# encryptorion-lab/phantom-fhe

Measured on AMD Instinct MI355X. Metric: forward NTT limb-transforms/s at N=2^16, 45 RNS moduli, higher is better.
Workload: dtype u64; 1 GPU; CKKS N=2^16, 45 data limbs (+15 special), forward NTT of a batch of 16 ciphertext polynomials per step (720 limb-transforms, 360 MiB, HBM-resident; configs[2] parameter set); N=65536, limbs=45, special_limbs=15, parallelism=ciphertext-batch x1, launch=K steps enqueued by one library call (2 K eager kernel launches)

## Files before the change

### phantom-fhe_amd/csrc/pha_ntt.hip

```cpp
#include "../../include/phantom_amd.h"
#include "pha_internal.h"
#include "pha_experiments.h"
#include "pha_ntt_core.h"

#include <atomic>
#include <type_traits>
#include <cstdlib>

namespace pha {

#ifndef PHA_X_HOIST_C
#define PHA_X_HOIST_C 0
#endif
#ifndef PHA_X_HOIST_S
#define PHA_X_HOIST_S 0
#endif
#ifndef PHA_X_VARIANT
#define PHA_X_VARIANT (1 | 32 | 64 | 2048 | 4096)
#endif
constexpr int kDefaultVariant = PHA_X_VARIANT;
#if defined(PHA_EXPERIMENTS)
std::atomic<int> g_ntt_variant{kDefaultVariant};
static inline int ntt_variant() { return g_ntt_variant.load(std::memory_order_relaxed); }
std::atomic<int> g_whole14_min{1 << 30};
std::atomic<int> g_fused_split{0};
std::atomic<int> g_fused_lag{2};
std::atomic<int> g_fused_min_tiles{1 << 30};
extern std::atomic<int> g_bconv_split;
#else
static constexpr int ntt_variant() { return kDefaultVariant; }
#endif
#if defined(PHA_EXP_STAMPS)
__device__ unsigned long long g_stamps[8];
__device__ unsigned long long g_wg_times[2048];
#endif

struct NttKArgs {
    const u64 *in;
    u64 *out;
    u64 *mid;
    const u64x2 *tw;
    const DModulus *mod;
    const u64x2 *ninv;
    const u64x2 *w1ninv;
    const u64 *twf;
    const u64x2 *ninvf, *w1ninvf;
    const FpInfo *fpinfo;
    const u64 *scale;
    const u64 *scale_shoup;
    const u64 *aux;
    const u64 *aux2;
    const u64 *scale2, *scale2_shoup;
    size_t aux2_stride;
    LimbSel sel;
    uint32_t log_n;
    uint32_t t1, t2;
    uint32_t active;
    uint32_t batch;
    size_t poly_stride, out_stride, aux_stride;
    size_t in_stride;
    bool first_pass_only;
    bool second_pass_only;
    bool first_pass_done;
    uint32_t excl_step, excl_limit, excl_mod;
    const u64 *pro_src;
    size_t pro_stride;
    uint32_t zfast_tiles;
    uint32_t zfast_run;
    u64 pro_t;
    size_t aux_pair_stride;
    const u64 *h_primes;
};

template <bool FWD, int EPI, bool FOLD>
__device__ __forceinline__ void tile_args(const NttKArgs &k, uint32_t twr, uint32_t tile, PassArgs &a) {
    const uint32_t prime = twr >= k.sel.remap_from ? twr + k.sel.remap_add : twr;
    const size_t n = (size_t)1 << k.log_n;
    a.in = k.in + (size_t)twr * n;
    a.out = k.out + (size_t)twr * n;
    a.tw = k.tw + (size_t)prime * n;
    a.twd = nullptr;
    a.q = k.mod[prime].value;
    a.tile = tile;
    a.rho0 = k.t1;
    a.stride = k.t2;
    if (!FWD && FOLD) {
        a.ninv = k.ninv[prime];
        a.w1ninv = k.w1ninv[prime];
    }
    a.pro_reduce = false;
    a.pro_ratio1 = 0;
    a.fp = false;
    if (k.fpinfo) {
        const FpInfo fi = k.fpinfo[prime];
        if (fi.ok) {
            a.fp = true;
            a.fpm = FpMod{fi.q, fi.qinv, (fi.ok & 2) != 0, (fi.ok & 4) != 0};
            a.twd = k.twf + (size_t)prime * n;
            if (!FWD && FOLD) {
                a.ninv = k.ninvf[prime];
                a.w1ninv = k.w1ninvf[prime];
// ... 6 lines not shown
    }
    a.aux = (EPI == EPI_FWD_MODDOWN || EPI == EPI_FWD_MODDOWN_ADD || EPI == EPI_FWD_KSRESCALE || EPI == EPI_INV_CANON_ADD) ? k.aux + (size_t)twr * n : nullptr;
    if (EPI == EPI_FWD_KSRESCALE) {
        a.scale2.x = k.scale2[twr];
        a.scale2.y = k.scale2_shoup[twr];
        a.aux2 = k.aux2 + (size_t)twr * n;
    }
}

#if defined(PHA_PASS_OCC)
#define PHA_PASS_ATTR __attribute__((amdgpu_waves_per_eu(PHA_PASS_OCC, PHA_PASS_OCC)))
#else
#define PHA_PASS_ATTR
#endif
#if defined(PHA_EXP_STAMPS)
#define PHA_STAMP(i) do { if (blockIdx.x == 0 && blockIdx.y == 0 && threadIdx.x == 0) g_stamps[i] = __builtin_readcyclecounter(); } while (0)
#else
#define PHA_STAMP(i) do { } while (0)
#endif

__device__ __forceinline__ bool limb_excluded(const NttKArgs &k, uint32_t twr, uint32_t z) {
    const uint32_t zd = k.excl_mod ? z % k.excl_mod : z;
    const uint32_t es = k.sel.excl_start + zd * k.excl_step;
    uint32_t ee = es + (k.sel.excl_end - k.sel.excl_start);
    ee = ee < k.excl_limit ? ee : k.excl_limit;
    return twr >= es && twr < ee;
}

template <class C, bool FWD, int EPI, bool FOLD>
__device__ __forceinline__ void full_tile_args(const NttKArgs &k, uint32_t twr, uint32_t z, uint32_t tile, PassArgs &a) {
    tile_args<FWD, EPI, FOLD>(k, twr, tile, a);
    if (k.batch > 1) {
        a.in += (size_t)z * k.in_stride;
        a.out += (size_t)z * k.out_stride;
        if (EPI == EPI_FWD_MODDOWN || EPI == EPI_FWD_MODDOWN_ADD || EPI == EPI_FWD_KSRESCALE) a.aux += (size_t)z * k.aux_stride;
        if (EPI == EPI_FWD_KSRESCALE) a.aux2 += (size_t)z * k.aux2_stride;
    }
    if (EPI == EPI_INV_CANON_ADD) a.aux += (size_t)(z >> 1) * k.aux_pair_stride + (size_t)(z & 1) * k.aux_stride;
    if (FWD && (C::STRIDED || C::WHOLE) && k.pro_src) {
        const uint32_t prime = twr >= k.sel.remap_from ? twr + k.sel.remap_add : twr;
        a.in = k.pro_src + (size_t)z * k.pro_stride;
        a.pro_reduce = true;
        a.pro_ratio1 = k.mod[prime].ratio1;
        a.pro_half = bfv_lift_threshold(k.pro_t);
        a.pro_inc = bfv_lift_increment(a.q, k.pro_t);
    }
}

template <class C, bool FWD, int EPI, bool FOLD, int HOIST, bool COH, int ONLY = 0, int PRO = PRO_NONE>
__device__ __forceinline__ void exec_pass(const PassArgs &a, u64 *lds, int tid) {
    u64 reg[C::EPT];
    u64x2 twreg[C::TW_TOTAL];
    using Prog = PassProgram<C, FWD, EPI, FOLD, HOIST, COH, PRO>;
    auto pass = [&](const PassArgs &pa) __attribute__((always_inline)) {
        Prog::load_twiddles(pa, tid, twreg);
        Prog::template run<0>(pa, lds, tid, reg, twreg);
        PHA_STAMP(1);
        tile_sync<C>();
        PHA_STAMP(2);
        Prog::template run<1>(pa, lds, tid, reg, twreg);
        PHA_STAMP(3);
        if constexpr (Prog::NSEG >= 3) {
            tile_sync<C>();
            PHA_STAMP(4);
            Prog::template run<2>(pa, lds, tid, reg, twreg);
            PHA_STAMP(5);
        }
        if constexpr (Prog::NSEG == 4) {
            tile_sync<C>();
            Prog::template run<3>(pa, lds, tid, reg, twreg);
        }
    };
    if (ONLY != 2 && a.fp) {
        PassArgs b = a;
        b.fp = true;
        pass(b);
    } else {
        PassArgs b = a;
        b.fp = false;
        pass(b);
    }
}

struct ZloopMap {
    uint32_t n_int, n_fp;
    uint32_t zper;
    uint32_t tiles;
    uint32_t int_blocks;
    uint8_t limb[128];
};
template <class C, bool FWD, int EPI, bool FOLD>
__global__ __launch_bounds__(C::THREADS) void ntt_zloop_kernel(const NttKArgs k, const ZloopMap m) {
    static_assert(!C::WHOLE, "the batched form exists for the passes of the two-pass plans");
    extern __shared__ __attribute__((aligned(16))) unsigned char smem[];
    u64 *lds = reinterpret_cast<u64 *>(smem);
    __builtin_amdgcn_s_setprio(3);
    const int tid = threadIdx.x;
    uint32_t b = blockIdx.x;
    PassArgs a;
    if (b < m.int_blocks) {
        const uint32_t tile = b % m.tiles, rest = b / m.tiles, z = rest % k.batch, twr = k.sel.start + m.limb[rest / k.batch];
        if (limb_excluded(k, twr, z)) return;
        full_tile_args<C, FWD, EPI, FOLD>(k, twr, z, tile, a);
        exec_pass<C, FWD, EPI, FOLD, 0, false, 2>(a, lds, tid);
        return;
    }
    b -= m.int_blocks;
    const uint32_t tile = b % m.tiles, rest = b / m.tiles, zgroups = (k.batch + m.zper - 1) / m.zper;
    const uint32_t twr = k.sel.start + m.limb[m.n_int + rest / zgroups];
    const uint32_t z0 = (rest % zgroups) * m.zper, z1 = (z0 + m.zper < k.batch) ? z0 + m.zper : k.batch;
    full_tile_args<C, FWD, EPI, FOLD>(k, twr, z0, tile, a);
    using Prog = PassProgram<C, FWD, EPI, FOLD, 1, false>;
    a.fp = true;
    u64x2 twreg[C::TW_TOTAL];
    Prog::load_twiddles(a, tid, twreg);
    u64 regA[C::EPT], regB[C::EPT];
    auto args_of = [&](uint32_t z) __attribute__((always_inline)) {
        PassArgs b = a;
        const size_t dz = (size_t)(z - z0);
        b.in += dz * k.in_stride;
        b.out += dz * k.out_stride;
        if (EPI == EPI_FWD_MODDOWN || EPI == EPI_FWD_MODDOWN_ADD || EPI == EPI_FWD_KSRESCALE) b.aux += dz * k.aux_stride;
        if (EPI == EPI_FWD_KSRESCALE) b.aux2 += dz * k.aux2_stride;
        return b;
    };
    auto transform = [&](const PassArgs &b, u64 *reg) __attribute__((always_inline)) {
        Prog::template run_prefetched<0>(b, lds, tid, reg, twreg);
        tile_sync<C>();
        Prog::template run_prefetched<1>(b, lds, tid, reg, twreg);
        if constexpr (Prog::NSEG >= 3) {
            tile_sync<C>();
            Prog::template run_prefetched<2>(b, lds, tid, reg, twreg);
        }
        if constexpr (Prog::NSEG == 4) {
            tile_sync<C>();
            Prog::template run_prefetched<3>(b, lds, tid, reg, twreg);
        }
        tile_sync<C>();
    };
    auto next = [&](uint32_t z) __attribute__((always_inline)) {
        while (z < z1 && limb_excluded(k, twr, z)) z++;
        return z;
    };
    uint32_t z = next(z0);
    if (z >= z1) return;
    Prog::prefetch(args_of(z), tid, regA);
    __builtin_amdgcn_s_setprio(0);
    for (;;) {
        uint32_t zn = next(z + 1);
        if (zn < z1) Prog::prefetch(args_of(zn), tid, regB);
        transform(args_of(z), regA);
        if (zn >= z1) break;
        z = zn;
        zn = next(z + 1);
        if (zn < z1) Prog::prefetch(args_of(zn), tid, regA);
        transform(args_of(z), regB);
        if (zn >= z1) break;
        z = zn;
    }
}

#if defined(PHA_X_OCC_S) || defined(PHA_X_OCC_C)
#ifndef PHA_X_OCC_S
#define PHA_X_OCC_S 2
#endif
#ifndef PHA_X_OCC_C
#define PHA_X_OCC_C 1
#endif
template <class C> constexpr int x_occ() { return C::WHOLE ? 1 : C::STRIDED ? (C::THREADS >= 512 ? PHA_X_OCC_S : 1) : (C::THREADS == 64 ? PHA_X_OCC_C : 1); }
#define PHA_PASS_BOUNDS __launch_bounds__(C::THREADS, x_occ<C>())
#else
#define PHA_PASS_BOUNDS __launch_bounds__(C::THREADS)
#endif
template <class C, bool FWD, int EPI, bool FOLD, int HOIST, int PRO = PRO_NONE>
__global__ PHA_PASS_BOUNDS PHA_PASS_ATTR void ntt_pass_kernel(const NttKArgs k) {
    extern __shared__ __attribute__((aligned(16))) unsigned char smem[];
    u64 *lds = reinterpret_cast<u64 *>(smem);

    __builtin_amdgcn_s_setprio(3);
    uint32_t tile = blockIdx.x, y = blockIdx.y, z = blockIdx.z;
    if (k.zfast_tiles) {
        const uint32_t b = blockIdx.x, per_chunk = k.zfast_run * k.batch, chunk = b / per_chunk, rem = b - chunk * per_chunk;
        z = rem / k.zfast_run;
        const uint32_t group = chunk * k.zfast_run + (rem - z * k.zfast_run);
        if (group >= k.zfast_tiles * k.sel.count) return;
        tile = group % k.zfast_tiles;
        y = group / k.zfast_tiles;
    }
    const uint32_t twr = k.sel.start + y;
    if (limb_excluded(k, twr, z)) return;
    PassArgs a;
    full_tile_args<C, FWD, EPI, FOLD>(k, twr, z, tile, a);
#if defined(PHA_EXP_STAMPS)
    const unsigned long long wg_t0 = wall_clock64();
#endif
    PHA_STAMP(0);
    exec_pass<C, FWD, EPI, FOLD, HOIST, false, 0, PRO>(a, lds, threadIdx.x);
#if defined(PHA_EXP_STAMPS)
    __builtin_amdgcn_s_waitcnt(0);
    PHA_STAMP(6);
    if (threadIdx.x == 0) {
        const unsigned id = blockIdx.y * gridDim.x + blockIdx.x;
        if (id < 1024) { g_wg_times[2 * id] = wg_t0; g_wg_times[2 * id + 1] = wall_clock64(); }
    }
#endif
}

#if defined(PHA_EXPERIMENTS)
#ifndef PHA_FUSED_MIN_WAVES
#define PHA_FUSED_MIN_WAVES 6
#endif
#if defined(PHA_FUSED_DEBUG)
__device__ uint32_t g_fused_dbg[8];
#endif
struct FusedArgs {
    uint32_t *cls;
    uint32_t *flags;
    uint32_t units, slots, tpl, lag, count;
    uint32_t active_units;
    uint32_t split;
};
__device__ __forceinline__ void l2_arrive(uint32_t *p) {
    asm volatile("global_atomic_add %0, %1, off" ::"v"(p), "v"(1u) : "memory");
}
__device__ __forceinline__ uint32_t l2_fetch_or(uint32_t *p, uint32_t v) {
    uint32_t r;
    asm volatile("global_atomic_or %0, %1, %2, off sc0\n\ts_waitcnt vmcnt(0)" : "=&v"(r) : "v"(p), "v"(v) : "memory");
    return r;
}
__device__ __forceinline__ uint32_t l2_fetch_add(uint32_t *p, uint32_t v) {
    uint32_t r;
    asm volatile("global_atomic_add %0, %1, %2, off sc0\n\ts_waitcnt vmcnt(0)" : "=&v"(r) : "v"(p), "v"(v) : "memory");
    return r;
}
__device__ __forceinline__ void l2_store(uint32_t *p, uint32_t v) {
    asm volatile("global_atomic_swap %0, %1, off" ::"v"(p), "v"(v) : "memory");
}

template <class C, bool FWD, int EPI, bool FOLD, bool COH>
__device__ __forceinline__ void fused_run_tile(const NttKArgs &k, uint32_t twr, uint32_t z, uint32_t tile, u64 *lds) {
    static_assert(C::THREADS == 512 || C::THREADS == 64, "the one-launch transform runs 512-thread workgroups");
    PassArgs a;
    if constexpr (C::THREADS == 512) {
        full_tile_args<C, FWD, EPI, FOLD>(k, twr, z, tile, a);
        exec_pass<C, FWD, EPI, FOLD, 0, COH>(a, lds, threadIdx.x);
    } else {
        const uint32_t wave = threadIdx.x >> 6;
        full_tile_args<C, FWD, EPI, FOLD>(k, twr, z, tile * 8 + wave, a);
        exec_pass<C, FWD, EPI, FOLD, 0, COH>(a, lds + (size_t)wave * C::LDS_WORDS, threadIdx.x & 63);
    }
}

template <class PS, class PC, bool FWD, int EPI, bool FOLD>
__global__ __launch_bounds__(512, PHA_FUSED_MIN_WAVES) void ntt_fused_kernel(const NttKArgs kA, const NttKArgs kB, const FusedArgs f) {
    extern __shared__ __attribute__((aligned(16))) unsigned char smem[];
    u64 *lds = reinterpret_cast<u64 *>(smem);
    const uint32_t b = blockIdx.x, xcd = b & 7u, within = b >> 3;
    const uint32_t role = f.split ? (within & 1u) : 2u, idx = f.split ? (within >> 1) : within;
    const uint32_t tile = idx % f.tpl, slot = idx / f.tpl;
    const uint32_t uA = slot * 8 + xcd;
    const bool has_a = role != 1u && slot < f.slots && uA < f.units && !limb_excluded(kA, kA.sel.start + uA % f.count, uA / f.count);
    const uint32_t uB = (slot - f.lag) * 8 + xcd;
    const bool has_b = role != 0u && slot >= f.lag && uB < f.units && !limb_excluded(kB, kB.sel.start + uB % f.count, uB / f.count);
    if (!has_a && !has_b) return;
    uint32_t cls_seen = 0, cls_mine = 0;
    if (threadIdx.x == 0) {
        uint32_t id;
        asm volatile("s_getreg_b32 %0, hwreg(HW_REG_XCC_ID)" : "=s"(id));
        cls_mine = (id & 7u) + 1;
        uint32_t expected = 0;
        __hip_atomic_compare_exchange_strong(f.cls + xcd, &expected, cls_mine, __ATOMIC_RELAXED, __ATOMIC_RELAXED, __HIP_MEMORY_SCOPE_AGENT);
        cls_seen = expected;
    }
    if (has_a) {
        const uint32_t z = uA / f.count, twr = kA.sel.start + uA % f.count;
        if (FWD) fused_run_tile<PS, true, EPI_NONE, false, false>(kA, twr, z, tile, lds);
        else fused_run_tile<PC, false, EPI_NONE, false, false>(kA, twr, z, tile, lds);
        asm volatile("s_waitcnt vmcnt(0)" ::: "memory");
        __syncthreads();
        if (threadIdx.x == 0) l2_arrive(f.flags + 2 * (size_t)uA);
    }
    if (threadIdx.x == 0 && cls_seen != 0 && cls_seen != cls_mine) {
#if defined(PHA_FUSED_DEBUG)
        if (atomicAdd(&g_fused_dbg[0], 1u) == 0) { g_fused_dbg[1] = b; g_fused_dbg[2] = cls_mine; g_fused_dbg[3] = cls_seen; }
#else
        __builtin_trap();
#endif
    }
    if (!has_b) return;
    const uint32_t z = uB / f.count, twr = kB.sel.start + uB % f.count;
    uint32_t *flag = f.flags + 2 * (size_t)uB;
    constexpr bool kWaveConsumer = FWD && PC::THREADS == 64;
    const bool poller = kWaveConsumer && f.split ? (threadIdx.x & 63) == 0 : threadIdx.x == 0;
    if (poller) {
        uint32_t spins = 0;
        while (l2_fetch_or(flag, 0u) < f.tpl) {
            __builtin_amdgcn_s_sleep(8);
#if defined(PHA_FUSED_DEBUG)
            if (++spins > (1u << 16)) { atomicAdd(&g_fused_dbg[4], 1u); break; }
#else
            if (++spins > (1u << 24)) __builtin_trap();
#endif
        }
    }
    if (!(kWaveConsumer && f.split)) __syncthreads();
    if (FWD) fused_run_tile<PC, true, EPI, false, true>(kB, twr, z, tile, lds);
    else fused_run_tile<PS, false, EPI, FOLD, true>(kB, twr, z, tile, lds);
    __syncthreads();
    if (threadIdx.x == 0 && __hip_atomic_fetch_add(flag + 1, 1u, __ATOMIC_RELAXED, __HIP_MEMORY_SCOPE_WORKGROUP) == f.tpl - 1) {
        l2_store(flag, 0u);
        l2_store(flag + 1, 0u);
        if (__hip_atomic_fetch_add(f.cls + 8, 1u, __ATOMIC_RELAXED, __HIP_MEMORY_SCOPE_AGENT) == f.active_units - 1) {
            for (int i = 0; i < 9; i++) __hip_atomic_store(f.cls + i, 0u, __ATOMIC_RELAXED, __HIP_MEMORY_SCOPE_AGENT);
        }
    }
}

#endif

template <class C, bool FWD, int EPI, bool FOLD, int PRO = PRO_NONE>
static void launch_pass(const NttKArgs &k, hipStream_t s) {
    const size_t n = (size_t)1 << k.log_n;
    const size_t lds_bytes = (size_t)C::LDS_WORDS * sizeof(u64);
    const unsigned tiles_per_limb = (unsigned)(n >> C::LOGTILE);
    dim3 grid(tiles_per_limb, k.sel.count, k.batch);
    NttKArgs kk = k;
    kk.zfast_tiles = 0;
    if (!C::STRIDED && !C::WHOLE && k.zfast_tiles) {
        kk.zfast_tiles = tiles_per_limb;
        kk.zfast_run = 8;
#if defined(PHA_X_KNOBS)
        static const unsigned run_x = std::getenv("PHA_X_ZRUN") ? (unsigned)std::atol(std::getenv("PHA_X_ZRUN")) : 8u;
        kk.zfast_run = run_x;
#endif
        const unsigned groups = tiles_per_limb * k.sel.count;
        grid = dim3(((groups + kk.zfast_run - 1) / kk.zfast_run) * kk.zfast_run * k.batch, 1, 1);
    }
    if (lds_bytes > 64 * 1024) {
        static std::atomic<uint64_t> raised{0};
        int dev = 0;
        PHA_HIP(hipGetDevice(&dev));
        const uint64_t bit = 1ull << (dev & 63);
        if (!(raised.load(std::memory_order_acquire) & bit)) {
            PHA_HIP(hipFuncSetAttribute(reinterpret_cast<const void *>(&ntt_pass_kernel<C, FWD, EPI, FOLD, (C::WHOLE ? 0 : C::STRIDED ? PHA_X_HOIST_S : PHA_X_HOIST_C), PRO>),
                                        hipFuncAttributeMaxDynamicSharedMemorySize, (int)lds_bytes));
            raised.fetch_or(bit, std::memory_order_release);
        }
    }
    constexpr int HX = C::WHOLE ? 0 : C::STRIDED ? PHA_X_HOIST_S : PHA_X_HOIST_C;
#if defined(PHA_X_KNOBS)
    static const size_t pad_s = std::getenv("PHA_X_LDS_S") ? (size_t)std::atol(std::getenv("PHA_X_LDS_S")) : 0;
    static const size_t pad_c = std::getenv("PHA_X_LDS_C") ? (size_t)std::atol(std::getenv("PHA_X_LDS_C")) : 0;
    const size_t lds_x = lds_bytes + (C::STRIDED ? pad_s : pad_c);
    hipLaunchKernelGGL((ntt_pass_kernel<C, FWD, EPI, FOLD, HX, PRO>), grid, dim3(C::THREADS), lds_x, s, kk);
#else
    hipLaunchKernelGGL((ntt_pass_kernel<C, FWD, EPI, FOLD, HX, PRO>), grid, dim3(C::THREADS), lds_bytes, s, kk);
#endif
    check_launch();
}

#if defined(PHA_EXPERIMENTS)
template <class PS, class PC, bool FWD, int EPI, bool FOLD>
static bool launch_fused(Context &c, const NttKArgs &kA_in, const NttKArgs &kB_in, hipStream_t s) {
    static_assert(PS::THREADS == 512 && PS::LOGTILE == 12, "strided pass: one 4096-coefficient tile per 512-thread workgroup");
    NttKArgs kA = kA_in, kB = kB_in;
    const size_t n = (size_t)1 << kA.log_n;
    kA.zfast_tiles = kB.zfast_tiles = 0;
    FusedArgs f{};
    f.count = kA.sel.count;
    f.units = kA.sel.count * kA.batch;
    f.slots = (f.units + 7) / 8;
    f.tpl = (uint32_t)(n >> 12);
    f.lag = (uint32_t)g_fused_lag.load(std::memory_order_relaxed);
    f.cls = c.ntt_flags(s, f.units);
    if (!f.cls) return false;
    f.flags = f.cls + 16;
    f.active_units = 0;
    for (uint32_t z = 0; z < kA.batch; z++) {
        const uint32_t zd = kA.excl_mod ? z % kA.excl_mod : z;
        const uint32_t es = kA.sel.excl_start + zd * kA.excl_step;
        uint32_t ee = es + (kA.sel.excl_end - kA.sel.excl_start);
        ee = ee < kA.excl_limit ? ee : kA.excl_limit;
        const uint32_t lo = es > kA.sel.start ? es : kA.sel.start;
        const uint32_t hi = ee < kA.sel.start + kA.sel.count ? ee : kA.sel.start + kA.sel.count;
        f.active_units += kA.sel.count - (hi > lo ? hi - lo : 0);
    }
    if (f.active_units == 0) return true;
    const size_t lds_a = (size_t)PS::LDS_WORDS * sizeof(u64);
    const size_t lds_b = (size_t)PC::LDS_WORDS * sizeof(u64) * (PC::THREADS == 64 ? 8 : 1);
    const size_t lds_bytes = lds_a > lds_b ? lds_a : lds_b;
    f.split = g_fused_split.load(std::memory_order_relaxed) ? 1u : 0u;
    const unsigned blocks = (f.slots + f.lag) * f.tpl * 8 * (f.split ? 2u : 1u);
    hipLaunchKernelGGL((ntt_fused_kernel<PS, PC, FWD, EPI, FOLD>), dim3(blocks), dim3(512), lds_bytes, s, kA, kB, f);
    check_launch();
    return true;
}

#endif

template <class P>
static void launch_inverse_last(const NttKArgs &k, int epi, hipStream_t s) {
    if (epi == EPI_INV_SCALE) launch_pass<P, false, EPI_INV_SCALE, true>(k, s);
    else if (epi == EPI_INV_CANON_ADD) launch_pass<P, false, EPI_INV_CANON_ADD, true>(k, s);
    else launch_pass<P, false, EPI_INV_CANON, true>(k, s);
}

template <class W>
static void forward_whole(NttKArgs k, int epi, hipStream_t s) {
    k.t1 = 1;
    k.t2 = W::T;
    k.mid = k.out;
    if (epi == EPI_FWD_MODDOWN) launch_pass<W, true, EPI_FWD_MODDOWN, false>(k, s);
    else if (epi == EPI_FWD_MODDOWN_ADD) launch_pass<W, true, EPI_FWD_MODDOWN_ADD, false>(k, s);
    else if (epi == EPI_FWD_KSRESCALE) launch_pass<W, true, EPI_FWD_KSRESCALE, false>(k, s);
    else if (k.pro_t) launch_pass<W, true, EPI_FWD_CANON, false, PRO_LIFT>(k, s);
    else launch_pass<W, true, EPI_FWD_CANON, false>(k, s);
}
template <class W>
static void inverse_whole(NttKArgs k, int epi, hipStream_t s) {
    k.t1 = 1;
    k.t2 = W::T;
    k.mid = k.out;
    launch_inverse_last<W>(k, epi, s);
}

#ifndef PHA_ZLOOP_MIN_BATCH
#define PHA_ZLOOP_MIN_BATCH 8
#endif
template <class C, bool FWD, int EPI, bool FOLD>
static bool launch_zloop(const NttKArgs &k, hipStream_t s) {
    if (k.batch < (uint32_t)PHA_ZLOOP_MIN_BATCH || k.pro_src) return false;
    const size_t n = (size_t)1 << k.log_n;
    const unsigned tiles_per_limb = (unsigned)(n >> C::LOGTILE);
    const size_t waves_per_poly = (size_t)tiles_per_limb * k.sel.count * (C::THREADS / 64);
    const size_t want = (size_t)256 * 4 * 4 * 3;
    uint32_t zper = (k.batch + ((k.batch + 7) / 8) - 1) / ((k.batch + 7) / 8);
    while (zper > 4 && waves_per_poly * ((k.batch + zper - 1) / zper) < want) zper = (zper + 1) / 2;
    if (waves_per_poly * ((k.batch + zper - 1) / zper) < want / 3) return false;
#if defined(PHA_X_KNOBS)
    static const unsigned zper_x = std::getenv("PHA_X_ZPER") ? (unsigned)std::atol(std::getenv("PHA_X_ZPER")) : 0u;
    if (zper_x) zper = zper_x;
#endif
    auto is_fp = [&](uint32_t y) {
        const uint32_t twr = k.sel.start + y, prime = twr >= k.sel.remap_from ? twr + k.sel.remap_add : twr;
        return k.fpinfo != nullptr && (k.h_primes[prime] >> 50) == 0;
    };
    if (k.sel.count > 128) return false;
    ZloopMap m{};
    m.zper = zper;
    m.tiles = tiles_per_limb;
    for (uint32_t y = 0; y < k.sel.count; y++)
        if (!is_fp(y)) m.limb[m.n_int++] = (uint8_t)y;
    for (uint32_t y = 0; y < k.sel.count; y++)
        if (is_fp(y)) m.limb[m.n_int + m.n_fp++] = (uint8_t)y;
    if (m.n_fp * 2 < k.sel.count) return false;
    m.int_blocks = m.n_int * tiles_per_limb * k.batch;
    NttKArgs kk = k;
    kk.zfast_tiles = 0;
    const unsigned blocks = m.int_blocks + m.n_fp * tiles_per_limb * ((k.batch + zper - 1) / zper);
    const size_t lds_bytes = (size_t)C::LDS_WORDS * sizeof(u64);
    hipLaunchKernelGGL((ntt_zloop_kernel<C, FWD, EPI, FOLD>), dim3(blocks), dim3(C::THREADS), lds_bytes, s, kk, m);
    check_launch();
    return true;
}

#ifndef PHA_IP_PLAN
#define PHA_IP_PLAN 3
#endif
template <int LOGN, int VARIANT>
static void forward_impl(NttKArgs k, int epi, hipStream_t s, Context *fused = nullptr) {
    using P1 = typename NttPlan<LOGN, VARIANT>::P1;
    using P2 = typename NttPlan<LOGN, VARIANT>::P2;
    k.t1 = P1::T;
    k.t2 = P2::T;
    if (k.first_pass_done && !(LOGN == 16 && VARIANT == 10 && P1::LOGT == 6))
        throw std::logic_error("ntt_forward: first_pass_done needs the 64 x 1024 plan the fused conversion wrote");
    u64 *const final_out = k.out;
    const size_t final_stride = k.out_stride;
    k.out = k.mid;
    k.out_stride = k.poly_stride;
    const NttKArgs k1 = k;
    k.in = k.mid;
    k.in_stride = k.poly_stride;
    k.out = final_out;
    k.out_stride = final_stride;
    k.pro_src = nullptr;
#if defined(PHA_EXPERIMENTS)
    if constexpr (P1::THREADS == 512 && P1::LOGTILE == 12 && P2::THREADS == 64) {
        if (fused && epi != EPI_FWD_KSRESCALE && !k.first_pass_done && !k.pro_t) {
            const bool done = epi == EPI_FWD_MODDOWN ? launch_fused<P1, P2, true, EPI_FWD_MODDOWN, false>(*fused, k1, k, s)
                              : epi == EPI_FWD_MODDOWN_ADD ? launch_fused<P1, P2, true, EPI_FWD_MODDOWN_ADD, false>(*fused, k1, k, s)
                                                           : launch_fused<P1, P2, true, EPI_FWD_CANON, false>(*fused, k1, k, s);
            if (done) return;
        }
    }
#else
    (void)fused;
#endif
    if (k.first_pass_done) {
    } else if (k1.pro_t) launch_pass<P1, true, EPI_NONE, false, PRO_LIFT>(k1, s);
    else launch_pass<P1, true, EPI_NONE, false>(k1, s);
    if (k.first_pass_only) return;
#if !defined(PHA_NO_ZLOOP)
    if constexpr (VARIANT == 10 || VARIANT == 3 || VARIANT == 4) {
        using Z2 = typename NttPlan<LOGN, VARIANT == 4 ? 3 : VARIANT>::P2;
        const bool done = epi == EPI_FWD_MODDOWN ? launch_zloop<Z2, true, EPI_FWD_MODDOWN, false>(k, s)
                          : epi == EPI_FWD_MODDOWN_ADD ? launch_zloop<Z2, true, EPI_FWD_MODDOWN_ADD, false>(k, s)
                          : epi == EPI_FWD_KSRESCALE ? launch_zloop<Z2, true, EPI_FWD_KSRESCALE, false>(k, s)
                                                     : launch_zloop<Z2, true, EPI_FWD_CANON, false>(k, s);
        if (done) return;
    }
#endif
    if (epi == EPI_FWD_MODDOWN) launch_pass<P2, true, EPI_FWD_MODDOWN, false>(k, s);
    else if (epi == EPI_FWD_MODDOWN_ADD) launch_pass<P2, true, EPI_FWD_MODDOWN_ADD, false>(k, s);
    else if (epi == EPI_FWD_KSRESCALE) launch_pass<P2, true, EPI_FWD_KSRESCALE, false>(k, s);
    else launch_pass<P2, true, EPI_FWD_CANON, false>(k, s);
}

template <int LOGN, int VARIANT>
static void inverse_impl(NttKArgs k, int epi, hipStream_t s, Context *fused = nullptr) {
    using P1 = typename NttPlan<LOGN, VARIANT>::P1;
    using P2 = typename NttPlan<LOGN, VARIANT>::P2;
    k.t1 = P1::T;
    k.t2 = P2::T;
    u64 *const final_out = k.out;
    const size_t final_stride = k.out_stride;
    k.out = k.mid;
    k.out_stride = k.poly_stride;
    const NttKArgs k1 = k;
    k.in = k.mid;
    k.in_stride = k.poly_stride;
    k.out = final_out;
    k.out_stride = final_stride;
#if defined(PHA_EXPERIMENTS)
    if constexpr (P1::THREADS == 512 && P1::LOGTILE == 12 && P2::THREADS == 64) {
        if (fused && epi != EPI_INV_CANON_ADD) {
            const bool done = epi == EPI_INV_SCALE ? launch_fused<P1, P2, false, EPI_INV_SCALE, true>(*fused, k1, k, s)
                                                   : launch_fused<P1, P2, false, EPI_INV_CANON, true>(*fused, k1, k, s);
            if (done) return;
        }
    }
#else
    (void)fused;
#endif
    if (k.second_pass_only) {
        using IpPlan = NttPlan<LOGN, (LOGN >= 14 && LOGN <= 16) ? PHA_IP_PLAN : 3>;
        if (P1::LOGT + IpPlan::P2::LOGT != LOGN)
            throw std::logic_error("second_pass_only: the chosen plan's strided pass does not complete the fused mod-up's contiguous pass");
        launch_inverse_last<P1>(k, epi, s);
        return;
    }
#if !defined(PHA_NO_ZLOOP)
    if constexpr (VARIANT == 10 || VARIANT == 3 || VARIANT == 4) {
        using Z2 = typename NttPlan<LOGN, VARIANT == 4 ? 3 : VARIANT>::P2;
        if (!launch_zloop<Z2, false, EPI_NONE, false>(k1, s)) launch_pass<P2, false, EPI_NONE, false>(k1, s);
        launch_inverse_last<P1>(k, epi, s);
        return;
    }
#endif
    launch_pass<P2, false, EPI_NONE, false>(k1, s);
    launch_inverse_last<P1>(k, epi, s);
}

static NttKArgs make_args(Context &c, const u64 *in, u64 *mid, u64 *out, const LimbSel &sel, const NttExtra &x,
                          bool fwd) {
    NttKArgs k{};
    k.in = in;
    k.mid = mid;
    k.out = out;
    k.tw = fwd ? c.d_tw.p : c.d_itw.p;
    k.mod = c.d_mod.p;
    k.ninv = c.d_ninv.p;
    k.w1ninv = c.d_w1ninv.p;
    const bool use_fp = !(ntt_variant() & 8);
    k.twf = fwd ? c.d_twf.p : c.d_itwf.p;
    k.ninvf = c.d_ninvf.p;
    k.w1ninvf = c.d_w1ninvf.p;
    k.fpinfo = use_fp ? c.d_fpinfo.p : nullptr;
    k.scale = x.scale;
    k.scale_shoup = x.scale_shoup;
    k.aux = x.aux;
    k.aux2 = x.aux2;
    k.scale2 = x.scale2;
    k.scale2_shoup = x.scale2_shoup;
    k.aux2_stride = x.aux2_stride ? x.aux2_stride : x.poly_stride;
    k.sel = sel;
    k.log_n = c.log_n;
    k.h_primes = c.primes.data();
    k.batch = x.batch ? x.batch : 1;
    k.poly_stride = x.poly_stride;
    k.in_stride = x.in_stride ? x.in_stride : x.poly_stride;
    k.first_pass_only = fwd && x.first_pass_only;
    k.second_pass_only = !fwd && x.second_pass_only;
    k.first_pass_done = fwd && x.first_pass_done;
    k.out_stride = x.out_stride ? x.out_stride : x.poly_stride;
    k.aux_stride = x.aux_stride ? x.aux_stride : x.poly_stride;
    k.excl_step = x.excl_step;
    k.excl_limit = x.excl_limit;
    k.excl_mod = x.excl_mod;
    k.pro_src = fwd ? x.pro_src : nullptr;
    k.pro_stride = x.pro_stride;
    k.pro_t = fwd && x.pro_src ? x.pro_lift_t : 0;
    k.aux_pair_stride = x.aux_pair_stride;
    uint32_t excl = 0;
    if (sel.excl_end > sel.excl_start) {
        const uint32_t lo = sel.excl_start > sel.start ? sel.excl_start : sel.start;
        const uint32_t hi = sel.excl_end < sel.start + sel.count ? sel.excl_end : sel.start + sel.count;
        excl = hi > lo ? hi - lo : 0;
        if (excl && (lo != sel.excl_start || hi != sel.excl_end)) excl = 0xffffffffu;
    }
    k.active = excl == 0xffffffffu ? 0 : sel.count - excl;
    return k;
}

static void check_sel(Context &c, const LimbSel &sel) {
    if (sel.count == 0) return;
    const uint32_t last = sel.start + sel.count - 1;
    const uint32_t prime_last = last >= sel.remap_from ? last + sel.remap_add : last;
    if (prime_last >= c.rows) throw std::invalid_argument("modulus index out of range of the NTT tables");
}


template <class C, int BETA, bool FP>
__device__ __forceinline__ void modup_ip_body(const NttKArgs &k, const ModupIpArgs &ip, uint32_t twr, uint32_t prime, uint32_t tile,
                                              u64 *lds, int tid) {
    constexpr int RL = C::NR - 1, r = C::r(RL), K = 1 << r, G = C::EPT >> r;
    static_assert(C::LOGT - C::s0(RL) - r == 0, "the last round holds runs of K consecutive coefficients");
    using Prog = PassProgram<C, true, EPI_NONE, false, 0, false>;
    const size_t n = (size_t)1 << k.log_n;
    const DModulus m = k.mod[prime];
    const u64 q = m.value;
    FpMod fm{};
    u64 accb[C::EPT], acca[C::EPT];
#pragma unroll
    for (int i = 0; i < C::EPT; i++) accb[i] = acca[i] = FP ? as_u64(0.0) : 0;
    size_t g0[G];
#pragma unroll
    for (int gi = 0; gi < G; gi++) {
        int v, hi, lo;
// ... 815 lines not shown
```

### phantom-fhe_amd/csrc/pha_ntt_core.h

```cpp
#pragma once
#include "pha_arith.h"
#include "pha_bfv_lift.h"

namespace pha {

constexpr int kTileElems = 4096;

enum Epilogue {
    EPI_NONE = 0,
    EPI_FWD_CANON = 1,
    EPI_FWD_MODDOWN = 2,
    EPI_INV_CANON = 3,
    EPI_INV_SCALE = 4,
    EPI_FWD_MODDOWN_ADD = 5,
    EPI_FWD_KSRESCALE = 6,
    EPI_INV_CANON_ADD = 7,
};

enum Prologue {
    PRO_NONE = 0,
    PRO_LIFT = 1,
};

template <int LOGT_, bool STRIDED_, int R0_, int R1_, int R2_ = 0, int EPT_ = 16, bool OT_ = false, int LOGTILE_ = 12,
// ... 658 lines not shown
        }
#if !defined(PHA_X_NOCOMPUTE)
        round_compute<C, RI, FWD, FOLD && RI == 0, fp_sched().recentre[SEG], fp_sched().full[SEG]>(a, tid, reg, twreg);
#endif
        if (last) fp_before_global_store(a, reg);
        round_out<C, RI, last, last ? EPI : (int)EPI_NONE>(a, lds, tid, reg);
    }

    template <int SEG>
    PHA_HD static void run_keep(const PassArgs &a, u64 *lds, int tid, u64 *reg, u64x2 *twreg) {
        constexpr int RI = FWD ? SEG : C::NR - 1 - SEG;
        static_assert(SEG == C::NR - 1 && SEG > 0, "run_keep is the last segment of a multi-round pass");
        segment_twiddles<SEG>(a, tid, twreg);
        round_load<C, RI, false, COH>(a, lds, tid, reg);
        round_compute<C, RI, FWD, FOLD && RI == 0>(a, tid, reg, twreg);
    }

    static constexpr int RI_FIRST = FWD ? 0 : C::NR - 1;
    PHA_HD static void prefetch(const PassArgs &a, int tid, u64 *reg) {
        round_load<C, RI_FIRST, true>(a, nullptr, tid, reg);
    }
    template <int SEG>
    PHA_HD static void run_prefetched(const PassArgs &a, u64 *lds, int tid, u64 *reg, u64x2 *twreg) {
        constexpr int RI = FWD ? SEG : C::NR - 1 - SEG;
        constexpr bool first = SEG == 0, last = SEG == C::NR - 1;
        segment_twiddles<SEG>(a, tid, twreg);
        if (!first) round_load<C, RI, false>(a, lds, tid, reg);
        if (first) fp_after_global_load(a, reg);
        round_compute<C, RI, FWD, FOLD && RI == 0, fp_sched().recentre[SEG], fp_sched().full[SEG]>(a, tid, reg, twreg);
        if (last) fp_before_global_store(a, reg);
        round_out<C, RI, last, last ? EPI : (int)EPI_NONE>(a, lds, tid, reg);
    }
};

template <int LOGN, int VARIANT> struct NttPlan;
template <> struct NttPlan<12, 0> { using P1 = PassCfg<6, true, 3, 3>;  using P2 = PassCfg<6, false, 3, 3>; };
template <> struct NttPlan<13, 0> { using P1 = PassCfg<6, true, 3, 3>;  using P2 = PassCfg<7, false, 4, 3>; };
template <> struct NttPlan<14, 0> { using P1 = PassCfg<7, true, 4, 3>;  using P2 = PassCfg<7, false, 4, 3>; };
template <> struct NttPlan<15, 0> { using P1 = PassCfg<7, true, 4, 3>;  using P2 = PassCfg<8, false, 4, 4>; };
template <> struct NttPlan<16, 0> { using P1 = PassCfg<8, true, 4, 4>;  using P2 = PassCfg<8, false, 4, 4>; };
template <> struct NttPlan<17, 0> { using P1 = PassCfg<8, true, 4, 4>;  using P2 = PassCfg<9, false, 3, 3, 3>; };
template <> struct NttPlan<12, 1> { using P1 = PassCfg<6, true, 3, 3, 0, 8>;  using P2 = PassCfg<6, false, 3, 3, 0, 8>; };
template <> struct NttPlan<13, 1> { using P1 = PassCfg<6, true, 3, 3, 0, 8>;  using P2 = PassCfg<7, false, 3, 2, 2, 8>; };
template <> struct NttPlan<14, 1> { using P1 = PassCfg<7, true, 3, 2, 2, 8>;  using P2 = PassCfg<7, false, 3, 2, 2, 8>; };
template <> struct NttPlan<15, 1> { using P1 = PassCfg<7, true, 3, 2, 2, 8>;  using P2 = PassCfg<8, false, 3, 3, 2, 8>; };
template <> struct NttPlan<16, 1> { using P1 = PassCfg<8, true, 3, 3, 2, 8>;  using P2 = PassCfg<8, false, 3, 3, 2, 8>; };
template <> struct NttPlan<17, 1> { using P1 = PassCfg<8, true, 3, 3, 2, 8>;  using P2 = PassCfg<9, false, 3, 3, 3, 8>; };
template <> struct NttPlan<12, 2> { using P1 = PassCfg<6, true, 3, 3, 0, 8>;  using P2 = PassCfg<6, false, 3, 3, 0, 8, true>; };
template <> struct NttPlan<13, 2> { using P1 = PassCfg<6, true, 3, 3, 0, 8>;  using P2 = PassCfg<7, false, 3, 2, 2, 8, true>; };
template <> struct NttPlan<14, 2> { using P1 = PassCfg<7, true, 3, 2, 2, 8>;  using P2 = PassCfg<7, false, 3, 2, 2, 8, true>; };
template <> struct NttPlan<15, 2> { using P1 = PassCfg<7, true, 3, 2, 2, 8>;  using P2 = PassCfg<8, false, 3, 3, 2, 8, true>; };
template <> struct NttPlan<16, 2> { using P1 = PassCfg<8, true, 3, 3, 2, 8>;  using P2 = PassCfg<8, false, 3, 3, 2, 8, true>; };
template <> struct NttPlan<17, 2> { using P1 = PassCfg<8, true, 3, 3, 2, 8>;  using P2 = PassCfg<9, false, 3, 3, 3, 8, true>; };
template <> struct NttPlan<12, 3> { using P1 = PassCfg<6, true, 3, 3, 0, 8>;  using P2 = PassCfg<6, false, 3, 3, 0, 8, false, 9>; };
template <> struct NttPlan<13, 3> { using P1 = PassCfg<6, true, 3, 3, 0, 8>;  using P2 = PassCfg<7, false, 3, 2, 2, 8, false, 9>; };
template <> struct NttPlan<14, 3> { using P1 = PassCfg<7, true, 3, 2, 2, 8>;  using P2 = PassCfg<7, false, 3, 2, 2, 8, false, 9>; };
template <> struct NttPlan<15, 3> { using P1 = PassCfg<7, true, 3, 2, 2, 8>;  using P2 = PassCfg<8, false, 3, 3, 2, 8, false, 9>; };
template <> struct NttPlan<16, 3> { using P1 = PassCfg<8, true, 3, 3, 2, 8>;  using P2 = PassCfg<8, false, 3, 3, 2, 8, false, 9>; };
template <> struct NttPlan<17, 3> { using P1 = PassCfg<8, true, 3, 3, 2, 8>;  using P2 = PassCfg<9, false, 3, 3, 3, 8, false, 9>; };
template <> struct NttPlan<12, 4> { using P1 = PassCfg<6, true, 3, 3, 0, 8>;  using P2 = PassCfg<6, false, 3, 3, 0, 8, true, 9>; };
template <> struct NttPlan<13, 4> { using P1 = PassCfg<6, true, 3, 3, 0, 8>;  using P2 = PassCfg<7, false, 3, 2, 2, 8, true, 9>; };
template <> struct NttPlan<14, 4> { using P1 = PassCfg<7, true, 3, 2, 2, 8>;  using P2 = PassCfg<7, false, 3, 2, 2, 8, true, 9>; };
template <> struct NttPlan<15, 4> { using P1 = PassCfg<7, true, 3, 2, 2, 8>;  using P2 = PassCfg<8, false, 3, 3, 2, 8, true, 9>; };
template <> struct NttPlan<16, 4> { using P1 = PassCfg<8, true, 3, 3, 2, 8>;  using P2 = PassCfg<8, false, 3, 3, 2, 8, true, 9>; };
template <> struct NttPlan<17, 4> { using P1 = PassCfg<8, true, 3, 3, 2, 8>;  using P2 = PassCfg<9, false, 3, 3, 3, 8, true, 9>; };
template <> struct NttPlan<14, 5> { using P1 = PassCfg<7, true, 3, 2, 2, 8>;  using P2 = PassCfg<7, false, 2, 2, 2, 4, false, 8, false, 1>; };
template <> struct NttPlan<15, 5> { using P1 = PassCfg<7, true, 3, 2, 2, 8>;  using P2 = PassCfg<8, false, 2, 2, 2, 4, false, 8, false, 2>; };
template <> struct NttPlan<16, 5> { using P1 = PassCfg<8, true, 3, 3, 2, 8>;  using P2 = PassCfg<8, false, 2, 2, 2, 4, false, 8, false, 2>; };
template <> struct NttPlan<14, 6> { using P1 = PassCfg<7, true, 2, 2, 2, 4, false, 11, false, 1>;  using P2 = NttPlan<14, 5>::P2; };
template <> struct NttPlan<15, 6> { using P1 = PassCfg<7, true, 2, 2, 2, 4, false, 11, false, 1>;  using P2 = NttPlan<15, 5>::P2; };
template <> struct NttPlan<16, 6> { using P1 = PassCfg<8, true, 2, 2, 2, 4, false, 11, false, 2>;  using P2 = NttPlan<16, 5>::P2; };
template <> struct NttPlan<14, 7> { using P1 = PassCfg<7, true, 2, 2, 2, 4, false, 12, false, 1>;  using P2 = NttPlan<14, 5>::P2; };
template <> struct NttPlan<15, 7> { using P1 = PassCfg<7, true, 2, 2, 2, 4, false, 12, false, 1>;  using P2 = NttPlan<15, 5>::P2; };
template <> struct NttPlan<16, 7> { using P1 = PassCfg<8, true, 2, 2, 2, 4, false, 12, false, 2>;  using P2 = NttPlan<16, 5>::P2; };
template <> struct NttPlan<16, 8> { using P1 = PassCfg<7, true, 3, 2, 2, 8>;  using P2 = PassCfg<9, false, 3, 3, 3, 8, false, 9>; };
template <> struct NttPlan<16, 9> { using P1 = PassCfg<7, true, 3, 2, 2, 8>;  using P2 = PassCfg<9, false, 3, 3, 3, 8, true, 9>; };
template <> struct NttPlan<16, 10> { using P1 = PassCfg<6, true, 3, 3, 0, 8, false, 11>;  using P2 = PassCfg<10, false, 3, 3, 2, 8, false, 10, false, 2>; };
template <> struct NttPlan<16, 12> { using P1 = PassCfg<6, true, 3, 3, 0, 8>;  using P2 = PassCfg<10, false, 4, 3, 3, 16, false, 10>; };
template <> struct NttPlan<16, 13> { using P1 = PassCfg<6, true, 2, 2, 2, 4, false, 10>;  using P2 = NttPlan<16, 10>::P2; };
using WholePlan12 = PassCfg<12, false, 4, 4, 4, 16, false, 12, true>;
using WholePlan13 = PassCfg<13, false, 4, 4, 4, 16, false, 13, true, 1>;
using WholePlan14 = PassCfg<14, false, 4, 4, 4, 16, false, 14, true, 2>;

}
```

Before: 2.589 million NTT/s.

## Reverse strided-pass block order so the zloop pass reuses cache-resident limbs

Adds a PassOrder descriptor that remaps the first (strided) pass grid so blocks run limbs and batch entries in the reverse of the order the following zloop pass consumes them. The most recently written data is then still in the last-level cache when the second pass starts reading it. An optional mode splits the limbs into two halves when the working set exceeds the cache size, though it is off by default. The cost is an extra kernel argument plus decode work in the pass kernel, and block scheduling may become less balanced.

```diff
diff --git a/phantom-fhe_amd/csrc/pha_ntt.hip b/phantom-fhe_amd/csrc/pha_ntt.hip
--- a/phantom-fhe_amd/csrc/pha_ntt.hip
+++ b/phantom-fhe_amd/csrc/pha_ntt.hip
@@ -17,6 +17,12 @@
 #endif
 #ifndef PHA_X_VARIANT
 #define PHA_X_VARIANT (1 | 32 | 64 | 2048 | 4096)
+#endif
+#ifndef PHA_NTT_PASS_ORDER
+#define PHA_NTT_PASS_ORDER 1
+#endif
+#ifndef PHA_NTT_ORDER_INT_HEAD
+#define PHA_NTT_ORDER_INT_HEAD 1
 #endif
 constexpr int kDefaultVariant = PHA_X_VARIANT;
 #if defined(PHA_EXPERIMENTS)
@@ -189,13 +195,6 @@
     }
 }
 
-struct ZloopMap {
-    uint32_t n_int, n_fp;
-    uint32_t zper;
-    uint32_t tiles;
-    uint32_t int_blocks;
-    uint8_t limb[128];
-};
 template <class C, bool FWD, int EPI, bool FOLD>
 __global__ __launch_bounds__(C::THREADS) void ntt_zloop_kernel(const NttKArgs k, const ZloopMap m) {
     static_assert(!C::WHOLE, "the batched form exists for the passes of the two-pass plans");
@@ -280,7 +279,7 @@
 #define PHA_PASS_BOUNDS __launch_bounds__(C::THREADS)
 #endif
 template <class C, bool FWD, int EPI, bool FOLD, int HOIST, int PRO = PRO_NONE>
-__global__ PHA_PASS_BOUNDS PHA_PASS_ATTR void ntt_pass_kernel(const NttKArgs k) {
+__global__ PHA_PASS_BOUNDS PHA_PASS_ATTR void ntt_pass_kernel(const NttKArgs k, const PassOrder o) {
     extern __shared__ __attribute__((aligned(16))) unsigned char smem[];
     u64 *lds = reinterpret_cast<u64 *>(smem);
 
@@ -294,6 +293,11 @@
         tile = group % k.zfast_tiles;
         y = group / k.zfast_tiles;
     }
+#if PHA_NTT_PASS_ORDER
+    else if (o.tiles) {
+        if (!pass_order_decode(o, k.batch, blockIdx.x, blockIdx.y, blockIdx.z, y, z, tile)) return;
+    }
+#endif
     const uint32_t twr = k.sel.start + y;
     if (limb_excluded(k, twr, z)) return;
     PassArgs a;
@@ -426,7 +430,7 @@
 #endif
 
 template <class C, bool FWD, int EPI, bool FOLD, int PRO = PRO_NONE>
-static void launch_pass(const NttKArgs &k, hipStream_t s) {
+static void launch_pass(const NttKArgs &k, hipStream_t s, const PassOrder *order = nullptr) {
     const size_t n = (size_t)1 << k.log_n;
     const size_t lds_bytes = (size_t)C::LDS_WORDS * sizeof(u64);
     const unsigned tiles_per_limb = (unsigned)(n >> C::LOGTILE);
@@ -443,6 +447,11 @@
         const unsigned groups = tiles_per_limb * k.sel.count;
         grid = dim3(((groups + kk.zfast_run - 1) / kk.zfast_run) * kk.zfast_run * k.batch, 1, 1);
     }
+    PassOrder o{};
+    if (order && !kk.zfast_tiles) {
+        o = *order;
+        pass_order_grid(o, k.batch, grid.x, grid.y, grid.z);
+    }
     if (lds_bytes > 64 * 1024) {
         static std::atomic<uint64_t> raised{0};
         int dev = 0;
@@ -459,9 +468,9 @@
     static const size_t pad_s = std::getenv("PHA_X_LDS_S") ? (size_t)std::atol(std::getenv("PHA_X_LDS_S")) : 0;
     static const size_t pad_c = std::getenv("PHA_X_LDS_C") ? (size_t)std::atol(std::getenv("PHA_X_LDS_C")) : 0;
     const size_t lds_x = lds_bytes + (C::STRIDED ? pad_s : pad_c);
-    hipLaunchKernelGGL((ntt_pass_kernel<C, FWD, EPI, FOLD, HX, PRO>), grid, dim3(C::THREADS), lds_x, s, kk);
+    hipLaunchKernelGGL((ntt_pass_kernel<C, FWD, EPI, FOLD, HX, PRO>), grid, dim3(C::THREADS), lds_x, s, kk, o);
 #else
-    hipLaunchKernelGGL((ntt_pass_kernel<C, FWD, EPI, FOLD, HX, PRO>), grid, dim3(C::THREADS), lds_bytes, s, kk);
+    hipLaunchKernelGGL((ntt_pass_kernel<C, FWD, EPI, FOLD, HX, PRO>), grid, dim3(C::THREADS), lds_bytes, s, kk, o);
 #endif
     check_launch();
 }
@@ -506,10 +515,10 @@
 #endif
 
 template <class P>
-static void launch_inverse_last(const NttKArgs &k, int epi, hipStream_t s) {
-    if (epi == EPI_INV_SCALE) launch_pass<P, false, EPI_INV_SCALE, true>(k, s);
-    else if (epi == EPI_INV_CANON_ADD) launch_pass<P, false, EPI_INV_CANON_ADD, true>(k, s);
-    else launch_pass<P, false, EPI_INV_CANON, true>(k, s);
+static void launch_inverse_last(const NttKArgs &k, int epi, hipStream_t s, const PassOrder *order = nullptr) {
+    if (epi == EPI_INV_SCALE) launch_pass<P, false, EPI_INV_SCALE, true>(k, s, order);
+    else if (epi == EPI_INV_CANON_ADD) launch_pass<P, false, EPI_INV_CANON_ADD, true>(k, s, order);
+    else launch_pass<P, false, EPI_INV_CANON, true>(k, s, order);
 }
 
 template <class W>
@@ -534,41 +543,50 @@
 #ifndef PHA_ZLOOP_MIN_BATCH
 #define PHA_ZLOOP_MIN_BATCH 8
 #endif
-template <class C, bool FWD, int EPI, bool FOLD>
-static bool launch_zloop(const NttKArgs &k, hipStream_t s) {
-    if (k.batch < (uint32_t)PHA_ZLOOP_MIN_BATCH || k.pro_src) return false;
+template <class C>
+static bool plan_zloop(const NttKArgs &k, ZloopMap &m) {
+    if (k.pro_src || k.sel.count > 128) return false;
     const size_t n = (size_t)1 << k.log_n;
     const unsigned tiles_per_limb = (unsigned)(n >> C::LOGTILE);
-    const size_t waves_per_poly = (size_t)tiles_per_limb * k.sel.count * (C::THREADS / 64);
-    const size_t want = (size_t)256 * 4 * 4 * 3;
-    uint32_t zper = (k.batch + ((k.batch + 7) / 8) - 1) / ((k.batch + 7) / 8);
-    while (zper > 4 && waves_per_poly * ((k.batch + zper - 1) / zper) < want) zper = (zper + 1) / 2;
-    if (waves_per_poly * ((k.batch + zper - 1) / zper) < want / 3) return false;
+    uint32_t zper = zloop_zper(k.batch, (size_t)tiles_per_limb * k.sel.count, C::THREADS / 64, PHA_ZLOOP_MIN_BATCH);
+    if (!zper) return false;
 #if defined(PHA_X_KNOBS)
     static const unsigned zper_x = std::getenv("PHA_X_ZPER") ? (unsigned)std::atol(std::getenv("PHA_X_ZPER")) : 0u;
     if (zper_x) zper = zper_x;
 #endif
-    auto is_fp = [&](uint32_t y) {
+    uint8_t fp[128];
+    for (uint32_t y = 0; y < k.sel.count; y++) {
         const uint32_t twr = k.sel.start + y, prime = twr >= k.sel.remap_from ? twr + k.sel.remap_add : twr;
-        return k.fpinfo != nullptr && (k.h_primes[prime] >> 50) == 0;
-    };
-    if (k.sel.count > 128) return false;
-    ZloopMap m{};
-    m.zper = zper;
-    m.tiles = tiles_per_limb;
-    for (uint32_t y = 0; y < k.sel.count; y++)
-        if (!is_fp(y)) m.limb[m.n_int++] = (uint8_t)y;
-    for (uint32_t y = 0; y < k.sel.count; y++)
-        if (is_fp(y)) m.limb[m.n_int + m.n_fp++] = (uint8_t)y;
-    if (m.n_fp * 2 < k.sel.count) return false;
-    m.int_blocks = m.n_int * tiles_per_limb * k.batch;
+        fp[y] = k.fpinfo != nullptr && (k.h_primes[prime] >> 50) == 0;
+    }
+    return zloop_fill(m, k.sel.count, fp, k.batch, zper, tiles_per_limb);
+}
+template <class C, bool FWD, int EPI, bool FOLD>
+static void launch_zloop(const NttKArgs &k, const ZloopMap &m, hipStream_t s) {
     NttKArgs kk = k;
     kk.zfast_tiles = 0;
-    const unsigned blocks = m.int_blocks + m.n_fp * tiles_per_limb * ((k.batch + zper - 1) / zper);
     const size_t lds_bytes = (size_t)C::LDS_WORDS * sizeof(u64);
-    hipLaunchKernelGGL((ntt_zloop_kernel<C, FWD, EPI, FOLD>), dim3(blocks), dim3(C::THREADS), lds_bytes, s, kk, m);
+    hipLaunchKernelGGL((ntt_zloop_kernel<C, FWD, EPI, FOLD>), dim3(zloop_blocks(m, k.batch)), dim3(C::THREADS), lds_bytes, s, kk, m);
     check_launch();
-    return true;
+}
+template <class C>
+static void launch_zloop_forward(const NttKArgs &k, const ZloopMap &m, int epi, hipStream_t s) {
+    if (epi == EPI_FWD_MODDOWN) launch_zloop<C, true, EPI_FWD_MODDOWN, false>(k, m, s);
+    else if (epi == EPI_FWD_MODDOWN_ADD) launch_zloop<C, true, EPI_FWD_MODDOWN_ADD, false>(k, m, s);
+    else if (epi == EPI_FWD_KSRESCALE) launch_zloop<C, true, EPI_FWD_KSRESCALE, false>(k, m, s);
+    else launch_zloop<C, true, EPI_FWD_CANON, false>(k, m, s);
+}
+
+constexpr size_t kLastLevelCacheBytes = (size_t)256 << 20;
+static NttKArgs limb_range(const NttKArgs &k, uint32_t lo, uint32_t cnt) {
+    NttKArgs h = k;
+    h.sel.start = k.sel.start + lo;
+    h.sel.count = cnt;
+    return h;
+}
+static uint32_t order_parts(const NttKArgs &k) {
+    const size_t bytes = ((size_t)k.sel.count * k.batch << k.log_n) * sizeof(u64);
+    return PHA_NTT_PASS_ORDER == 2 && k.sel.count >= 2 && bytes > kLastLevelCacheBytes ? 2u : 1u;
 }
 
 #ifndef PHA_IP_PLAN
@@ -604,20 +622,34 @@
 #else
     (void)fused;
 #endif
-    if (k.first_pass_done) {
-    } else if (k1.pro_t) launch_pass<P1, true, EPI_NONE, false, PRO_LIFT>(k1, s);
-    else launch_pass<P1, true, EPI_NONE, false>(k1, s);
-    if (k.first_pass_only) return;
+    auto strided = [&](const NttKArgs &ka, const PassOrder *order) {
+        if (ka.pro_t) launch_pass<P1, true, EPI_NONE, false, PRO_LIFT>(ka, s, order);
+        else launch_pass<P1, true, EPI_NONE, false>(ka, s, order);
+    };
 #if !defined(PHA_NO_ZLOOP)
     if constexpr (VARIANT == 10 || VARIANT == 3 || VARIANT == 4) {
         using Z2 = typename NttPlan<LOGN, VARIANT == 4 ? 3 : VARIANT>::P2;
-        const bool done = epi == EPI_FWD_MODDOWN ? launch_zloop<Z2, true, EPI_FWD_MODDOWN, false>(k, s)
-                          : epi == EPI_FWD_MODDOWN_ADD ? launch_zloop<Z2, true, EPI_FWD_MODDOWN_ADD, false>(k, s)
-                          : epi == EPI_FWD_KSRESCALE ? launch_zloop<Z2, true, EPI_FWD_KSRESCALE, false>(k, s)
-                                                     : launch_zloop<Z2, true, EPI_FWD_CANON, false>(k, s);
-        if (done) return;
-    }
-#endif
+        ZloopMap m;
+        if (!k.first_pass_only && plan_zloop<Z2>(k, m)) {
+            if (k.first_pass_done) return launch_zloop_forward<Z2>(k, m, epi, s);
+            if (PHA_NTT_PASS_ORDER == 0) {
+                strided(k1, nullptr);
+                return launch_zloop_forward<Z2>(k, m, epi, s);
+            }
+            const uint32_t parts = order_parts(k), cut = pass_order_half(k.sel.count);
+            for (uint32_t h = 0; h < parts; h++) {
+                const uint32_t lo = h * cut, hi = parts == 1 ? k.sel.count : h ? k.sel.count : cut;
+                const ZloopMap mh = parts == 1 ? m : zloop_sub(m, lo, hi, k.batch);
+                const PassOrder o = pass_order_reverse(mh, (uint32_t)(((size_t)1 << k.log_n) >> P1::LOGTILE), PHA_NTT_ORDER_INT_HEAD != 0);
+                strided(limb_range(k1, lo, hi - lo), &o);
+                launch_zloop_forward<Z2>(limb_range(k, lo, hi - lo), mh, epi, s);
+            }
+            return;
+        }
+    }
+#endif
+    if (!k.first_pass_done) strided(k1, nullptr);
+    if (k.first_pass_only) return;
     if (epi == EPI_FWD_MODDOWN) launch_pass<P2, true, EPI_FWD_MODDOWN, false>(k, s);
     else if (epi == EPI_FWD_MODDOWN_ADD) launch_pass<P2, true, EPI_FWD_MODDOWN_ADD, false>(k, s);
     else if (epi == EPI_FWD_KSRESCALE) launch_pass<P2, true, EPI_FWD_KSRESCALE, false>(k, s);
@@ -660,8 +692,25 @@
 #if !defined(PHA_NO_ZLOOP)
     if constexpr (VARIANT == 10 || VARIANT == 3 || VARIANT == 4) {
         using Z2 = typename NttPlan<LOGN, VARIANT == 4 ? 3 : VARIANT>::P2;
-        if (!launch_zloop<Z2, false, EPI_NONE, false>(k1, s)) launch_pass<P2, false, EPI_NONE, false>(k1, s);
-        launch_inverse_last<P1>(k, epi, s);
+        ZloopMap m;
+        if (!plan_zloop<Z2>(k1, m)) {
+            launch_pass<P2, false, EPI_NONE, false>(k1, s);
+            launch_inverse_last<P1>(k, epi, s);
+            return;
+        }
+        if (PHA_NTT_PASS_ORDER == 0) {
+            launch_zloop<Z2, false, EPI_NONE, false>(k1, m, s);
+            launch_inverse_last<P1>(k, epi, s);
+            return;
+        }
+        const uint32_t parts = order_parts(k), cut = pass_order_half(k.sel.count);
+        for (uint32_t h = 0; h < parts; h++) {
+            const uint32_t lo = h * cut, hi = parts == 1 ? k.sel.count : h ? k.sel.count : cut;
+            const ZloopMap mh = parts == 1 ? m : zloop_sub(m, lo, hi, k.batch);
+            const PassOrder o = pass_order_reverse(mh, (uint32_t)(((size_t)1 << k.log_n) >> P1::LOGTILE), PHA_NTT_ORDER_INT_HEAD != 0);
+            launch_zloop<Z2, false, EPI_NONE, false>(limb_range(k1, lo, hi - lo), mh, s);
+            launch_inverse_last<P1>(limb_range(k, lo, hi - lo), epi, s, &o);
+        }
         return;
     }
 #endif
diff --git a/phantom-fhe_amd/csrc/pha_ntt_core.h b/phantom-fhe_amd/csrc/pha_ntt_core.h
--- a/phantom-fhe_amd/csrc/pha_ntt_core.h
+++ b/phantom-fhe_amd/csrc/pha_ntt_core.h
@@ -764,4 +764,78 @@
 using WholePlan13 = PassCfg<13, false, 4, 4, 4, 16, false, 13, true, 1>;
 using WholePlan14 = PassCfg<14, false, 4, 4, 4, 16, false, 14, true, 2>;
 
-}
+struct ZloopMap {
+    uint32_t n_int, n_fp;
+    uint32_t zper;
+    uint32_t tiles;
+    uint32_t int_blocks;
+    uint8_t limb[128];
+};
+
+inline uint32_t zloop_zper(uint32_t batch, size_t wgs_per_poly, uint32_t waves_per_wg, uint32_t min_batch) {
+    if (batch < min_batch) return 0;
+    const size_t waves_per_poly = wgs_per_poly * waves_per_wg;
+    const size_t want = (size_t)256 * 4 * 4 * 3;
+    uint32_t zper = (batch + ((batch + 7) / 8) - 1) / ((batch + 7) / 8);
+    while (zper > 4 && waves_per_poly * ((batch + zper - 1) / zper) < want) zper = (zper + 1) / 2;
+    if (waves_per_poly * ((batch + zper - 1) / zper) < want / 3) return 0;
+    return zper;
+}
+
+inline bool zloop_fill(ZloopMap &m, uint32_t count, const uint8_t *fp, uint32_t batch, uint32_t zper, uint32_t tiles_per_limb) {
+    if (count > 128) return false;
+    m = ZloopMap{};
+    m.zper = zper;
+    m.tiles = tiles_per_limb;
+    for (uint32_t y = 0; y < count; y++)
+        if (!fp[y]) m.limb[m.n_int++] = (uint8_t)y;
+    for (uint32_t y = 0; y < count; y++)
+        if (fp[y]) m.limb[m.n_int + m.n_fp++] = (uint8_t)y;
+    if (m.n_fp * 2 < count) return false;
+    m.int_blocks = m.n_int * tiles_per_limb * batch;
+    return true;
+}
+inline uint32_t zloop_blocks(const ZloopMap &m, uint32_t batch) { return m.int_blocks + m.n_fp * m.tiles * ((batch + m.zper - 1) / m.zper); }
+
+inline ZloopMap zloop_sub(const ZloopMap &m, uint32_t lo, uint32_t hi, uint32_t batch) {
+    ZloopMap s{};
+    s.zper = m.zper;
+    s.tiles = m.tiles;
+    for (uint32_t i = 0; i < m.n_int + m.n_fp; i++) {
+        if (m.limb[i] < lo || m.limb[i] >= hi) continue;
+        s.limb[s.n_int + s.n_fp] = (uint8_t)(m.limb[i] - lo);
+        if (i < m.n_int) s.n_int++;
+        else s.n_fp++;
+    }
+    s.int_blocks = s.n_int * s.tiles * batch;
+    return s;
+}
+
+struct PassOrder {
+    uint32_t tiles;
+    uint32_t count;
+    uint32_t limb4[32];
+};
+PHA_HD uint32_t pass_order_limb(const PassOrder &o, uint32_t i) { return (o.limb4[i >> 2] >> ((i & 3u) * 8u)) & 0xffu; }
+inline PassOrder pass_order_reverse(const ZloopMap &m, uint32_t tiles_per_limb, bool int_head) {
+    PassOrder o{};
+    o.tiles = tiles_per_limb;
+    o.count = m.n_int + m.n_fp;
+    uint32_t at = 0;
+    auto put = [&](uint32_t y) { o.limb4[at >> 2] |= y << ((at & 3u) * 8u); at++; };
+    if (int_head)
+        for (uint32_t i = 0; i < m.n_int; i++) put(m.limb[i]);
+    for (uint32_t i = o.count; i-- > (int_head ? m.n_int : 0u);) put(m.limb[i]);
+    return o;
+}
+inline uint32_t pass_order_half(uint32_t count) { return (count + 1) / 2; }
+inline void pass_order_grid(const PassOrder &o, uint32_t batch, uint32_t &gx, uint32_t &gy, uint32_t &gz) { gx = o.tiles; gy = batch; gz = o.count; }
+PHA_HD bool pass_order_decode(const PassOrder &o, uint32_t batch, uint32_t bx, uint32_t by, uint32_t bz, uint32_t &y, uint32_t &z, uint32_t &tile) {
+    if (bx >= o.tiles || by >= batch || bz >= o.count) return false;
+    tile = bx;
+    z = batch - 1 - by;
+    y = pass_order_limb(o, bz);
+    return true;
+}
+
+}
```

Result: faster. 2.661 million NTT/s (median of 6 runs) (+2.8%).
